# Sudo42b/vision.cpp

Hardware: AMD Instinct MI355X
Metric: images/sec, Depth-Anything-V2-Small 518x518 f16 (higher is better)
Workload: dtype f16; 1 GPU; Depth-Anything-V2-Small f16 (DINOv2-S ViT) 518x518 batch=32 per MI355X (BASELINE.json configs[1]); global_batch=32, weights=random-init synthetic GGUF (seed 0), parallelism=dp1 (image shards, no data-path collective), hip_graph=True

## Files before the change

### vision.cpp_amd/csrc/kernels_block16.hip

```cpp
#include "vx_common.h"

#include <cstdlib>
#include <type_traits>
#include <utility>

namespace {

constexpr int D = 384, HID = 1536;
constexpr int NT = D / 16;
constexpr int KB = D / 32;
constexpr int FR = 24;
constexpr int SLAB = FR * 1024;
constexpr int N_OUT = NT / 2;
constexpr int N_MLP = 2 * (HID / 32);
constexpr int N_QKV = 3 * NT / 2;

constexpr int V_BO = 0, V_G2 = 768, V_B2 = 1152, V_B1 = 1536, V_BFC2 = 3072;
constexpr int V_GN = 3840, V_BN = 4224, V_BQKV = 4608;
constexpr int V_GF = 5760, V_BF = 6144;
constexpr int V_TOTAL = 6528;

#ifndef VISP_BLOCK16_PF
#define VISP_BLOCK16_PF 4
#endif
#ifndef VISP_BLOCK16_DEFER
#define VISP_BLOCK16_DEFER 1
#endif
#ifndef VISP_BLOCK16_DEFER_MLP
#define VISP_BLOCK16_DEFER_MLP 0
#endif
#ifndef VISP_BLOCK16_LN_FENCE
#define VISP_BLOCK16_LN_FENCE 1
#endif
#ifndef VISP_BLOCK16_SPREAD
#define VISP_BLOCK16_SPREAD 1
#endif
constexpr int LN_FENCE = VISP_BLOCK16_LN_FENCE;
constexpr int SPREAD = VISP_BLOCK16_SPREAD;
constexpr int PF = VISP_BLOCK16_PF;
constexpr int DG = VISP_BLOCK16_DEFER;
static_assert(PF % 2 == 0 && FR % PF == 0 && PF - 2 * DG >= 2, "the window must hold the deferred groups and the next step's first group");
constexpr int SMEM_RING = 4 * SLAB;
constexpr int SMEM_BYTES = SMEM_RING + V_TOTAL * 4;
constexpr int WP = 2 * FR / 8;

typedef unsigned int u32x4 __attribute__((ext_vector_type(4)));
typedef unsigned int u32x2 __attribute__((ext_vector_type(2)));

template <int... I, class F>
__device__ __forceinline__ void static_for_impl(std::integer_sequence<int, I...>, F&& f) { (f(std::integral_constant<int, I>{}), ...); }
template <int N, class F>
__device__ __forceinline__ void static_for(F&& f) { static_for_impl(std::make_integer_sequence<int, N>{}, f); }
#define CI(x) (decltype(x)::value)

__device__ __forceinline__ float row_sum4(float v) {
    v += __shfl_xor(v, 16, 64);
    v += __shfl_xor(v, 32, 64);
    return v;
}

__device__ __forceinline__ void lds_dma16(const void* gsrc, unsigned lds_dst) {
    unsigned keep;
    asm volatile("s_mov_b32 %0, m0\n\ts_mov_b32 m0, %2\n\ts_nop 0\n\tglobal_load_lds_dwordx4 %1, off\n\ts_mov_b32 m0, %0"
                 : "=&s"(keep) : "v"(gsrc), "s"(lds_dst) : "memory");
}

#ifndef VISP_BLOCK16_DBG
#define VISP_BLOCK16_DBG 0
#endif
constexpr int DBG = VISP_BLOCK16_DBG;
#ifndef VISP_BLOCK16_MID
#define VISP_BLOCK16_MID 5
#endif

template <bool MLP, bool QKV, bool TAP>
__global__ __launch_bounds__(512) void dino_block16_kernel(const vx_dino_block_args args) {
    float* const a_x = args.x; const void* const a_att = args.att; const void* const a_wmlp = args.w_mlp; const void* const a_wqkv = args.w_qkv;
    const float* const a_vmlp = args.vec_mlp; const float* const a_vqkv = args.vec_qkv; const float* const a_vtap = args.vec_tap;
    void* const a_feat = args.feat; void* const a_q = args.q; void* const a_k = args.k; void* const a_v = args.v; float* const a_cap = args.cap_x1;
    const int a_M = args.M, a_T = args.T, a_H = args.H;
    const float a_qs = args.q_scale, a_eps = args.eps;
    unsigned long long* const a_stamps = static_cast<unsigned long long*>(args.stamps);
    auto stamp = [&](int slot) __attribute__((always_inline)) {
        if (a_stamps && threadIdx.x == 0) a_stamps[(size_t)blockIdx.x * 16 + slot] = slot >= 14 ? __builtin_amdgcn_s_memrealtime() : __builtin_amdgcn_s_memtime();
    };
    stamp(0);
    stamp(14);

    extern __shared__ __attribute__((aligned(16))) unsigned char smem[];
    unsigned char* const ring = smem;
    float* const vec = reinterpret_cast<float*>(smem + SMEM_RING);

    const int tid = threadIdx.x, lane = tid & 63;
    const int wave = __builtin_amdgcn_readfirstlane(tid >> 6);
    const int n = lane & 15, g = lane >> 4;
    const int m = blockIdx.x * 128 + wave * 16 + n;

    constexpr int row_bytes_f32 = D * 4, row_bytes_f16 = D * 2;
    const __amdgpu_buffer_rsrc_t rs_x = __builtin_amdgcn_make_buffer_rsrc(a_x, 0, (int)((long)a_M * row_bytes_f32), 0x00020000);
    const unsigned xoff = m < a_M ? (unsigned)m * row_bytes_f32 + 16 * g : 0x80000000u;
    auto ld_x = [&](int T) __attribute__((always_inline)) -> f32x4 {
        return __builtin_bit_cast(f32x4, __builtin_amdgcn_raw_buffer_load_b128(rs_x, xoff, 64 * T, 0));
    };
    auto st_x = [&](int T, f32x4 v) __attribute__((always_inline)) {
        __builtin_amdgcn_raw_buffer_store_b128(__builtin_bit_cast(u32x4, v), rs_x, xoff, 64 * T, 0);
    };

    auto pair_src = [&](int k) __attribute__((always_inline)) -> const unsigned char* {
        constexpr int first_qkv = MLP ? N_OUT + N_MLP : 0;
        const unsigned char* base = (MLP && k < first_qkv) ? static_cast<const unsigned char*>(a_wmlp) + (size_t)k * SLAB
                                                          : static_cast<const unsigned char*>(a_wqkv) + (size_t)(k - first_qkv) * SLAB;
        return base + (wave * WP) * 1024 + lane * 16;
    };
    constexpr int n_slabs = (MLP ? N_OUT + N_MLP : 0) + (QKV ? N_QKV : 0);
    const unsigned ring_lds = (unsigned)(size_t)(lptr_t)ring;
    auto feed_pair = [&](int k, int stage) __attribute__((always_inline)) {
        if constexpr (DBG & 1) return;
        const unsigned char* src = pair_src(k);
        const unsigned dst = __builtin_amdgcn_readfirstlane(ring_lds + stage * SLAB + wave * WP * 1024);
#pragma unroll
        for (int z = 0; z < WP; ++z) lds_dma16(src + z * 1024, dst + z * 1024);
    };
    const unsigned char* owed_src = nullptr;
    unsigned owed_dst = 0;
    bool owed = false;
    auto feed_piece = [&](int z) __attribute__((always_inline)) {
        if constexpr (DBG & 1) return;
        if (owed) lds_dma16(owed_src + z * 1024, owed_dst + z * 1024);
    };
    const unsigned char* const rd0 = ring + lane * 16;
    {
        feed_pair(0, 0);
        if constexpr (MLP)
            for (int i = tid; i < 3840 / 4; i += 512) reinterpret_cast<float4*>(vec)[i] = reinterpret_cast<const float4*>(a_vmlp)[i];
        if constexpr (QKV)
            for (int i = tid; i < 1920 / 4; i += 512) reinterpret_cast<float4*>(vec + V_GN)[i] = reinterpret_cast<const float4*>(a_vqkv)[i];
        if constexpr (TAP)
            for (int i = tid; i < 768 / 4; i += 512) reinterpret_cast<float4*>(vec + V_GF)[i] = reinterpret_cast<const float4*>(a_vtap)[i];
    }

    stamp(1);
    if constexpr ((DBG & 4096) != 0) { if (wave >= 4) __builtin_amdgcn_s_barrier(); }
    int k = 0, st = 0;
    const unsigned char *curx = rd0, *cury = rd0 + SLAB;
    f16x8 wfx[PF] = {}, wfy[PF] = {};

    unsigned long long w_vm = 0, w_bar = 0, w_n = 0;
    auto boundary = [&](auto yc, auto nfill) __attribute__((always_inline)) {
        constexpr int YOUNGER = CI(yc);
        if constexpr (DBG & 1024) {
            const unsigned long long t0 = __builtin_amdgcn_s_memtime();
            wait_vmcnt<YOUNGER>();
            const unsigned long long t1 = __builtin_amdgcn_s_memtime();
            __syncthreads();
            const unsigned long long t2 = __builtin_amdgcn_s_memtime();
            w_vm += t1 - t0; w_bar += t2 - t1; w_n += 1;
        } else {
        wait_vmcnt<YOUNGER>();
        if constexpr (!(DBG & 64)) __syncthreads();
        }
        curx = rd0 + st * SLAB;
        cury = curx + SLAB;
        if constexpr (!(DBG & 8)) {
#pragma unroll
            for (int i = 0; i < CI(nfill); ++i) {
                wfx[i] = *reinterpret_cast<const f16x8*>(curx + i * 1024);
                wfy[i] = *reinterpret_cast<const f16x8*>(cury + i * 1024);
            }
        }
        if constexpr (SPREAD) {
            owed = k + 2 < n_slabs;
            if (owed) {
                owed_src = pair_src(k + 2);
                owed_dst = __builtin_amdgcn_readfirstlane(ring_lds + (st ^ 2) * SLAB + wave * WP * 1024);
            }
        } else {
            if (k + 2 < n_slabs) feed_pair(k + 2, st ^ 2);
        }
        st ^= 2;
        k += 2;
    };
    auto stepx = [&](auto&& xm, auto&& ym, auto&& side, auto coldc, auto contc, auto yo, auto yc) __attribute__((always_inline)) {
        constexpr bool COLD = CI(coldc) != 0, CONT = CI(contc) != 0 && DG > 0;
        if constexpr (COLD || DG == 0) boundary(yo, std::integral_constant<int, PF>{});
        static_for<FR / 2>([&](auto gc) __attribute__((always_inline)) {
            constexpr int gi = CI(gc), f0 = 2 * gi, f1 = f0 + 1;
            if constexpr (CONT && gi == FR / 2 - DG) boundary(yc, std::integral_constant<int, PF - 2 * DG>{});
            if constexpr ((DBG & 2048) != 0 && gi == VISP_BLOCK16_MID) __builtin_amdgcn_s_barrier();
            ym(std::integral_constant<int, f1>{}, wfy[f1 % PF]);
            xm(std::integral_constant<int, f1>{}, wfx[f1 % PF]);
            ym(std::integral_constant<int, f0>{}, wfy[f0 % PF]);
            xm(std::integral_constant<int, f0>{}, wfx[f0 % PF]);
            constexpr int r0 = f0 + PF < FR ? f0 + PF : (CONT && gi >= FR / 2 - DG ? f0 + PF - FR : -1);
            if constexpr (r0 >= 0 && !(DBG & 8)) {
                wfx[f0 % PF] = *reinterpret_cast<const f16x8*>(curx + r0 * 1024);
                wfy[f0 % PF] = *reinterpret_cast<const f16x8*>(cury + r0 * 1024);
                wfx[f1 % PF] = *reinterpret_cast<const f16x8*>(curx + (r0 + 1) * 1024);
                wfy[f1 % PF] = *reinterpret_cast<const f16x8*>(cury + (r0 + 1) * 1024);
            }
            if constexpr (SPREAD && gi < WP) feed_piece(gi);
            side(std::integral_constant<int, 2 * f0>{});
            side(std::integral_constant<int, 2 * f0 + 1>{});
            side(std::integral_constant<int, 2 * f0 + 2>{});
            side(std::integral_constant<int, 2 * f0 + 3>{});
            __builtin_amdgcn_sched_barrier(0);
        });
    };
    constexpr std::integral_constant<int, 1> yes{};
    auto no_side = [](auto) {};
    constexpr std::integral_constant<int, 0> none{};

    auto vec4 = [&](const float* v, int T) __attribute__((always_inline)) -> f32x4 {
        const float4 q = *reinterpret_cast<const float4*>(v + 16 * T + 4 * g);
        f32x4 c = {q.x, q.y, q.z, q.w};
        return c;
    };
    auto mfma = [](const f16x8& w, const f16x8& b, f32x4 c) __attribute__((always_inline)) -> f32x4 {
        return __builtin_amdgcn_mfma_f32_16x16x32_f16(w, b, c, 0, 0, 0);
// ... 379 lines not shown
```

### vision.cpp_amd/csrc/kernels_gemm.hip

```cpp
#include "vx_common.h"

#include <algorithm>

extern "C" int vx_gemm_f16_raw(const vx_gemm_args* args, void* stream);

namespace {

constexpr int BK = 64;
constexpr int WAVE = 64;

__device__ __attribute__((aligned(16))) unsigned char g_zero_page[64];

constexpr bool epi_is_f16_tile(int epi) {
    return epi == VX_EPI_F16 || epi == VX_EPI_F16_GELU || epi == VX_EPI_F16_RELU || epi == VX_EPI_F16_ADD ||
           epi == VX_EPI_QKV || epi == VX_EPI_PIXSHUF || epi == VX_EPI_HEAD_OUT || epi == VX_EPI_LRELU_AGC ||
           epi == VX_EPI_SILU;
}

template <int BM, int BN, int WM, int WN, int STAGES, int EPI, bool CONV>
__global__ __launch_bounds__(64 * (BM / WM) * (BN / WN)) void gemm_kernel(const vx_gemm_args p) {
    constexpr int WAVES_N = BN / WN;
    constexpr int MI = WM / 32, NI = WN / 32;
    constexpr int NWAVES = (BM / WM) * WAVES_N;
    constexpr int THREADS = WAVE * NWAVES;
    constexpr int A_INSTR = BM / (8 * NWAVES);
    constexpr int B_INSTR = BN / (8 * NWAVES);
    static_assert(A_INSTR >= 1 && B_INSTR >= 1 && (128 * (BN / 8)) % THREADS == 0 && THREADS >= BM, "tile / wave layout");

    constexpr int STAGE_BYTES = (BM + BN) * BK * 2;
    constexpr int LOADS = A_INSTR + B_INSTR;
    extern __shared__ __attribute__((aligned(16))) unsigned char smem[];

    const int tid = threadIdx.x, lane = tid & 63;
    const int wave = __builtin_amdgcn_readfirstlane(tid >> 6);
    unsigned long long* const stamps = reinterpret_cast<unsigned long long*>(p.debug_stamps);
    auto stamp = [&](int slot) {
        if (stamps && tid == 0) stamps[(size_t)blockIdx.x * 8 + slot] = __builtin_amdgcn_s_memtime();
    };
    stamp(0);
    if (stamps && tid == 0) stamps[(size_t)blockIdx.x * 8 + 6] = __builtin_amdgcn_s_memrealtime();
    const int wr = wave / WAVES_N, wc = wave % WAVES_N;
    const int r = lane & 31, h = lane >> 5;

    const int n_tiles_n = p.N / BN;
    int tile;
    {
        const int nwg = gridDim.x, b = blockIdx.x;
        const int q = nwg >> 3, rem = nwg & 7, xcd = b & 7;
        tile = (xcd < rem ? xcd * (q + 1) : rem * (q + 1) + (xcd - rem) * q) + (b >> 3);
    }
    int ks = 0;
    if (p.k_splits > 1) {
        const int n_tiles = gridDim.x / p.k_splits;
        ks = tile / n_tiles;
        tile -= ks * n_tiles;
    }
    const int tile_m = tile / n_tiles_n, tile_n = tile - tile_m * n_tiles_n;
    const int m0 = tile_m * BM, n0 = tile_n * BN;
    int kbase = 0, nk = p.K / BK;
    if (p.k_splits > 1) {
        const int per = (nk + p.k_splits - 1) / p.k_splits;
        kbase = ks * per;
        nk = min(per, nk - kbase);
    }

    float* const s_bias = reinterpret_cast<float*>(smem + STAGES * STAGE_BYTES);
    float* const s_lambda = s_bias + BN;
    int* const s_pix = reinterpret_cast<int*>(s_lambda + BN);
    if constexpr (EPI == VX_EPI_F16_ADD) {
        if (p.win_ws > 0 && tid < BM) {
            const int m = m0 + tid;
            int pix = -1;
            if (m < p.M) {
                const int ws = p.win_ws, rw = p.win_res, rh = p.win_res_h > 0 ? p.win_res_h : p.win_res, N = ws * ws;
                const int nwx = (rw + ws - 1) / ws, nwy = (rh + ws - 1) / ws;
                const int in = m % N;
                int wq = m / N;
                const int wx = wq % nwx;
                wq /= nwx;
                const int wy = wq % nwy, bb = wq / nwy;
                int py = wy * ws + in / ws + p.win_shift, px = wx * ws + in % ws + p.win_shift;
                if (py >= nwy * ws) py -= nwy * ws;
                if (px >= nwx * ws) px -= nwx * ws;
                if (py < rh && px < rw) pix = (bb * rh + py) * rw + px;
            }
            s_pix[tid] = pix;
        }
    }
    if (tid < BN) {
        s_bias[tid] = p.bias ? p.bias[n0 + tid] : 0.0f;
        if constexpr (EPI == VX_EPI_RESID_F32 || EPI == VX_EPI_HEAD_OUT) s_lambda[tid] = p.lambda[n0 + tid];
    }

    const f16* __restrict__ Ag = reinterpret_cast<const f16*>(p.A);
    const f16* __restrict__ Wg = reinterpret_cast<const f16*>(p.W);

    const int l_row = lane >> 3, l_pos = lane & 7;
    long a_off[A_INSTR];
    const long a_pix = CONV ? (p.conv_pix > 0 ? p.conv_pix : p.conv_Cin) : 0;
    int a_iy0[A_INSTR], a_ix0[A_INSTR], a_chunk[A_INSTR];
#pragma unroll
    for (int i = 0; i < A_INSTR; ++i) {
        const int row = (wave * A_INSTR + i) * 8 + l_row;
        a_chunk[i] = swz128(row, l_pos);
        int m = m0 + row;
        if constexpr (CONV) {
            if (m < p.M) {
                int ohw = p.conv_OH * p.conv_OW;
                int b = m / ohw, rm = m - b * ohw;
                int oy = rm / p.conv_OW, ox = rm - oy * p.conv_OW;
                a_off[i] = (long)b * p.conv_H * p.conv_W * a_pix;
                a_iy0[i] = oy * p.conv_stride - p.conv_pad;
                a_ix0[i] = ox * p.conv_stride - p.conv_pad;
            } else {
                a_off[i] = -1;
                a_iy0[i] = a_ix0[i] = 0;
            }
        } else {
            if (m >= p.M) m = p.M - 1;
            long arow = m;
            if (p.a_group > 0) arow = (long)(m / p.a_group) * p.a_group_stride + p.a_row_off + (m % p.a_group);
            a_off[i] = arow * p.lda;
            a_iy0[i] = a_ix0[i] = 0;
        }
    }
    long b_off[B_INSTR];
    int b_chunk[B_INSTR];
#pragma unroll
    for (int i = 0; i < B_INSTR; ++i) {
        const int row = (wave * B_INSTR + i) * 8 + l_row;
        b_chunk[i] = swz128(row, l_pos);
        b_off[i] = (long)(n0 + row) * p.K;
    }
    const int cin8 = CONV ? (p.conv_Cin >> 3) : 1;
    const int ntaps = CONV ? p.conv_kh * p.conv_kw : 1;

    auto issue_loads = [&](int kt, int stage) {
        unsigned char* const sa = smem + stage * STAGE_BYTES;
        unsigned char* const sb = sa + BM * BK * 2;
        const int k0 = (kbase + kt) * BK;
#pragma unroll
        for (int i = 0; i < A_INSTR; ++i) {
            const f16* src;
            if constexpr (CONV) {
                src = reinterpret_cast<const f16*>(g_zero_page);
                int kc = (k0 >> 3) + a_chunk[i];
                int tap = kc / cin8, c8 = kc - tap * cin8;
                if (a_off[i] >= 0 && tap < ntaps) {
                    int ky = tap / p.conv_kw, kx = tap - ky * p.conv_kw;
                    int iy = a_iy0[i] + ky, ix = a_ix0[i] + kx;
                    if ((unsigned)iy < (unsigned)p.conv_H && (unsigned)ix < (unsigned)p.conv_W)
                        src = Ag + a_off[i] + ((long)iy * p.conv_W + ix) * a_pix + c8 * 8;
                }
            } else {
                src = Ag + a_off[i] + k0 + a_chunk[i] * 8;
            }
            __builtin_amdgcn_global_load_lds((gptr_t)src, (lptr_t)(sa + (wave * A_INSTR + i) * 1024), 16, 0, 0);
        }
#pragma unroll
        for (int i = 0; i < B_INSTR; ++i)
            __builtin_amdgcn_global_load_lds((gptr_t)(Wg + b_off[i] + k0 + b_chunk[i] * 8),
                                             (lptr_t)(sb + (wave * B_INSTR + i) * 1024), 16, 0, 0);
    };

    f32x16 acc[MI][NI];
#pragma unroll
    for (int mi = 0; mi < MI; ++mi)
#pragma unroll
        for (int ni = 0; ni < NI; ++ni)
#pragma unroll
            for (int e = 0; e < 16; ++e) acc[mi][ni][e] = 0.0f;

    int f_off[BK / 16];
#pragma unroll
    for (int ks = 0; ks < BK / 16; ++ks) f_off[ks] = r * 128 + swz128(r, ks * 2 + h) * 16;

    auto compute = [&](int stage) {
        const unsigned char* const sa = smem + stage * STAGE_BYTES + wr * WM * 128;
        const unsigned char* const sb = smem + stage * STAGE_BYTES + BM * BK * 2 + wc * WN * 128;
        f16x8 af[2][MI], bf[2][NI];
        auto load_frags = [&](int ks, int set) {
#pragma unroll
            for (int mi = 0; mi < MI; ++mi) af[set][mi] = *reinterpret_cast<const f16x8*>(sa + f_off[ks] + mi * 32 * 128);
#pragma unroll
            for (int ni = 0; ni < NI; ++ni) bf[set][ni] = *reinterpret_cast<const f16x8*>(sb + f_off[ks] + ni * 32 * 128);
        };
        load_frags(0, 0);
#pragma unroll
        for (int ks = 0; ks < BK / 16; ++ks) {
            const int set = ks & 1;
            if (ks + 1 < BK / 16) load_frags(ks + 1, set ^ 1);
            __builtin_amdgcn_sched_barrier(0);
            if constexpr (CONV) {
                if (p.a_relu) {
#pragma unroll
                    for (int mi = 0; mi < MI; ++mi)
#pragma unroll
                        for (int j = 0; j < 8; ++j) af[set][mi][j] = af[set][mi][j] > (f16)0 ? af[set][mi][j] : (f16)0;
                }
            }
#pragma unroll
            for (int mi = 0; mi < MI; ++mi)
#pragma unroll
                for (int ni = 0; ni < NI; ++ni)
                    acc[mi][ni] = __builtin_amdgcn_mfma_f32_32x32x16_f16(bf[set][ni], af[set][mi], acc[mi][ni], 0, 0, 0);
        }
    };
    auto barrier = [&]() {
        wait_lgkmcnt0();
        __builtin_amdgcn_s_barrier();
        asm volatile("" ::: "memory");
    };

    stamp(1);
    if constexpr (STAGES == 1) {
        issue_loads(0, 0);
        for (int kt = 0; kt < nk; ++kt) {
            wait_vmcnt<0>();
            barrier();
            if (kt == 0) stamp(2);
            compute(0);
            barrier();
            if (kt + 1 < nk) issue_loads(kt + 1, 0);
        }
    } else {
#pragma unroll
        for (int s = 0; s < STAGES - 1; ++s)
            if (s < nk) issue_loads(s, s);
        int stage = 0;
        for (int kt = 0; kt < nk; ++kt) {
            const int ahead = min(STAGES - 2, nk - 1 - kt);
            if (ahead >= 2) wait_vmcnt<2 * LOADS>();
            else if (ahead == 1) wait_vmcnt<LOADS>();
            else wait_vmcnt<0>();
            barrier();
            int next_stage = stage == 0 ? STAGES - 1 : stage - 1;
            if (kt + STAGES - 1 < nk) issue_loads(kt + STAGES - 1, next_stage);
            compute(stage);
            stage = stage + 1 == STAGES ? 0 : stage + 1;
        }
        barrier();
    }

    const int n_valid = p.n_valid > 0 ? p.n_valid : p.N;
    stamp(3);

    if (p.k_splits > 1) {
        float* const part = p.k_partial + (long)ks * p.M * p.N;
#pragma unroll
        for (int mi = 0; mi < MI; ++mi) {
            const int m = m0 + wr * WM + mi * 32 + r;
            if (m >= p.M) continue;
#pragma unroll
            for (int ni = 0; ni < NI; ++ni)
#pragma unroll
                for (int g = 0; g < 4; ++g) {
                    const float4 v = {acc[mi][ni][4 * g + 0], acc[mi][ni][4 * g + 1], acc[mi][ni][4 * g + 2], acc[mi][ni][4 * g + 3]};
                    *reinterpret_cast<float4*>(part + (long)m * p.N + n0 + wc * WN + ni * 32 + 8 * g + 4 * h) = v;
                }
        }
        return;
    }

    if constexpr (!epi_is_f16_tile(EPI)) {
#pragma unroll
        for (int mi = 0; mi < MI; ++mi) {
            const int m = m0 + wr * WM + mi * 32 + r;
            if (m >= p.M) continue;
            long row = m;
            int t = 0;
            if constexpr (EPI == VX_EPI_TOKENS) {
                int b = m / p.tokens_P;
                t = m - b * p.tokens_P;
                row = (long)b * (p.tokens_P + 1) + 1 + t;
            }
            float* xrow = reinterpret_cast<float*>(p.out) + row * p.ldo + n0;
            const float* add_row = nullptr;
            if constexpr (EPI == VX_EPI_RESID_F32) add_row = xrow;
            else add_row = p.pos + (long)(1 + t) * p.N + n0;
            float4 xin[NI][4];
#pragma unroll
            for (int ni = 0; ni < NI; ++ni)
#pragma unroll
                for (int g = 0; g < 4; ++g)
                    xin[ni][g] = *reinterpret_cast<const float4*>(add_row + wc * WN + ni * 32 + 8 * g + 4 * h);
#pragma unroll
            for (int ni = 0; ni < NI; ++ni) {
#pragma unroll
                for (int g = 0; g < 4; ++g) {
                    const int nl = wc * WN + ni * 32 + 8 * g + 4 * h;
                    const float4 bias = *reinterpret_cast<const float4*>(s_bias + nl);
                    float4 v = {acc[mi][ni][4 * g + 0] + bias.x, acc[mi][ni][4 * g + 1] + bias.y,
                                acc[mi][ni][4 * g + 2] + bias.z, acc[mi][ni][4 * g + 3] + bias.w};
                    float4 x = xin[ni][g];
                    if constexpr (EPI == VX_EPI_RESID_F32) {
                        const float4 lam = *reinterpret_cast<const float4*>(s_lambda + nl);
                        x.x += v.x * lam.x; x.y += v.y * lam.y; x.z += v.z * lam.z; x.w += v.w * lam.w;
                    } else {
                        x.x += v.x; x.y += v.y; x.z += v.z; x.w += v.w;
                    }
                    *reinterpret_cast<float4*>(xrow + nl) = x;
                }
            }
        }
    } else {
        constexpr int NCH16 = BN / 8;
        constexpr int PITCH = BN * 2;
        unsigned char* const st = smem;
        float out_scale = 1.0f;
        if constexpr (EPI == VX_EPI_QKV) out_scale = n0 < p.qkv_H * 64 ? p.q_scale : 1.0f;
        constexpr int MPP = (MI % 2 == 0 && BM / WM <= 2) ? 2 : 1;
        constexpr int PASSES = MI / MPP;
        constexpr int WPP = 32 * MPP;
        constexpr int STAGE_ROWS = (BM / WM) * WPP;
#pragma unroll
        for (int ps = 0; ps < PASSES; ++ps) {
        if (ps > 0) __syncthreads();
#pragma unroll
        for (int mp = 0; mp < MPP; ++mp) {
            const int mi = ps * MPP + mp;
            const int ml = wr * WPP + mp * 32 + r;
#pragma unroll
            for (int ni = 0; ni < NI; ++ni) {
#pragma unroll
                for (int g = 0; g < 4; ++g) {
                    const int nl = wc * WN + ni * 32 + 8 * g + 4 * h;
                    const float4 bias = *reinterpret_cast<const float4*>(s_bias + nl);
                    float v[4] = {acc[mi][ni][4 * g + 0] + bias.x, acc[mi][ni][4 * g + 1] + bias.y,
                                  acc[mi][ni][4 * g + 2] + bias.z, acc[mi][ni][4 * g + 3] + bias.w};
#pragma unroll
                    for (int j = 0; j < 4; ++j) {
                        if constexpr (EPI == VX_EPI_F16_GELU) v[j] = gelu_tanh(v[j]);
                        if constexpr (EPI == VX_EPI_F16_RELU || EPI == VX_EPI_HEAD_OUT) v[j] = fmaxf(v[j], 0.0f);
                        if constexpr (EPI == VX_EPI_F16_ADD) { if (p.relu) v[j] = fmaxf(v[j], 0.0f); }
                        if constexpr (EPI == VX_EPI_QKV) v[j] *= out_scale;
                        if constexpr (EPI == VX_EPI_SILU) v[j] = silu(v[j]);
                    }
                    if constexpr (EPI == VX_EPI_LRELU_AGC) {
                        const int m = m0 + wr * WM + ps * WPP + mp * 32 + r;
                        const float nz = (p.noise && m < p.M) ? p.noise[m % p.noise_hw] : 0.0f;
#pragma unroll
                        for (int j = 0; j < 4; ++j) {
                            const float t = v[j] + nz;
                            v[j] = fminf(fmaxf((t < 0.0f ? 0.2f * t : t) * 1.41421356f, -256.0f), 256.0f);
                        }
                    }
                    f16x4 o = {(f16)v[0], (f16)v[1], (f16)v[2], (f16)v[3]};
                    const int c8 = nl >> 2;
                    const int phys16 = (c8 >> 1) ^ (ml & (NCH16 - 1));
                    *reinterpret_cast<f16x4*>(st + ml * PITCH + phys16 * 16 + (c8 & 1) * 8) = o;
                }
            }
        }
        __syncthreads();
        if (ps == 0) stamp(4);
        constexpr int CHUNKS = STAGE_ROWS * NCH16;
        static_assert(CHUNKS % THREADS == 0, "staging read-out");
#pragma unroll
        for (int it = 0; it < CHUNKS / THREADS; ++it) {
            const int id = tid + it * THREADS;
            const int ml = id / NCH16, j = id % NCH16;
            const int m = m0 + (ml / WPP) * WM + ps * WPP + (ml % WPP), n = n0 + j * 8;
            if (m >= p.M || n >= n_valid) continue;
            f16x8 v = *reinterpret_cast<const f16x8*>(st + ml * PITCH + (j ^ (ml & (NCH16 - 1))) * 16);
            if constexpr (EPI == VX_EPI_HEAD_OUT) {
                float part = 0.0f;
#pragma unroll
                for (int q = 0; q < 8; ++q) part += (float)v[q] * s_lambda[j * 8 + q];
                part += __shfl_xor(part, 1, 64);
                part += __shfl_xor(part, 2, 64);
                if (j == 0) reinterpret_cast<float*>(p.out)[m] = fmaxf(part + p.head_bias, 0.0f) * p.head_scale;
            } else if constexpr (EPI == VX_EPI_F16 || EPI == VX_EPI_F16_GELU || EPI == VX_EPI_F16_RELU || EPI == VX_EPI_LRELU_AGC || EPI == VX_EPI_SILU) {
                if constexpr (EPI == VX_EPI_LRELU_AGC || EPI == VX_EPI_SILU) {
                    if (p.res1) {
                        const long ldr = (EPI == VX_EPI_SILU && p.ld_res1 > 0) ? p.ld_res1 : p.ldo;
                        const f16x8 a = *reinterpret_cast<const f16x8*>(reinterpret_cast<const f16*>(p.res1) + (long)m * ldr + n);
#pragma unroll
                        for (int q = 0; q < 8; ++q) v[q] = (f16)((float)v[q] + (float)a[q]);
                    }
                }
                *reinterpret_cast<f16x8*>(reinterpret_cast<f16*>(p.out) + (long)m * p.ldo + n) = v;
            } else if constexpr (EPI == VX_EPI_F16_ADD) {
                long o = (long)m * p.ldo + n;
                if (p.win_ws > 0) {
                    const int pix = s_pix[m - m0];
                    if (pix < 0) continue;
                    o = (long)pix * p.ldo + n;
                }
                if (p.res1) {
                    f16x8 a = *reinterpret_cast<const f16x8*>(reinterpret_cast<const f16*>(p.res1) + o);
                    if (p.res2) {
                        f16x8 b = *reinterpret_cast<const f16x8*>(reinterpret_cast<const f16*>(p.res2) + o);
#pragma unroll
                        for (int q = 0; q < 8; ++q) v[q] = (f16)((float)v[q] + (float)a[q] + (float)b[q]);
                    } else if (p.post_gelu) {
#pragma unroll
                        for (int q = 0; q < 8; ++q) v[q] = (f16)gelu_tanh((float)v[q] + (float)a[q]);
                    } else {
#pragma unroll
                        for (int q = 0; q < 8; ++q) v[q] = (f16)((float)v[q] + (float)a[q]);
                    }
                }
                *reinterpret_cast<f16x8*>(reinterpret_cast<f16*>(p.out) + o) = v;
            } else if constexpr (EPI == VX_EPI_QKV) {
                const int C = p.qkv_H * 64;
                const int which = n0 / C, cc = n - which * C;
                const int hh = cc >> 6, d = cc & 63;
                const int b0 = m0 / p.qkv_T;
                int b = b0 + (m >= (b0 + 1) * p.qkv_T ? 1 : 0);
                if (p.qkv_T < BM) b = m / p.qkv_T;
                const int t = m - b * p.qkv_T;
                f16* dst = reinterpret_cast<f16*>(which == 0 ? p.q : (which == 1 ? p.k : p.vt));
                *reinterpret_cast<f16x8*>(dst + (((long)b * p.qkv_H + hh) * p.qkv_T + t) * 64 + d) = v;
            } else if constexpr (EPI == VX_EPI_PIXSHUF) {
                const int s = p.ps_s;
                const int tap = n / p.ps_Cout, co = n - tap * p.ps_Cout;
                const int dy = tap / s, dx = tap - dy * s;
                const int hw = p.ps_H * p.ps_W;
                const int b = m / hw, rem = m - b * hw;
                const int y = rem / p.ps_W, x = rem - y * p.ps_W;
                const long o = (((long)b * p.ps_H * s + (y * s + dy)) * (p.ps_W * s) + (x * s + dx)) * p.ldo + co;
                *reinterpret_cast<f16x8*>(reinterpret_cast<f16*>(p.out) + o) = v;
            }
        }
        }
    }
    stamp(5);
    if (stamps && tid == 0) stamps[(size_t)blockIdx.x * 8 + 7] = __builtin_amdgcn_s_memrealtime();
}

template <int BM, int BN, int WM, int WN, int STAGES, int EPI, bool CONV>
int launch(const vx_gemm_args& a, hipStream_t s) {
    constexpr int ring = STAGES * (BM + BN) * BK * 2;
    constexpr int out_stage = epi_is_f16_tile(EPI) ? 128 * BN * 2 : 0;
    constexpr int smem = (ring > out_stage ? ring : out_stage) + 2 * BN * 4 + (EPI == VX_EPI_F16_ADD ? BM * 4 : 0);
    auto kern = gemm_kernel<BM, BN, WM, WN, STAGES, EPI, CONV>;
    if constexpr (smem > 48 * 1024) VX_CHECK(vx_ensure_dynamic_lds(reinterpret_cast<const void*>(kern), smem));
    int tiles_m = (a.M + BM - 1) / BM, tiles_n = a.N / BN;
    hipLaunchKernelGGL(kern, dim3(tiles_m * tiles_n * (a.k_splits > 1 ? a.k_splits : 1)), dim3(64 * (BM / WM) * (BN / WN)), smem, s, a);
    VX_LAUNCH_CHECK();
    return 1;
}

template <int EPI, bool CONV>
int dispatch_tile(const vx_gemm_args& a, hipStream_t s) {
    if (a.N % 128 == 0) {
        if constexpr (!CONV) {
            if (a.stages == 2) return launch<128, 128, 64, 64, 2, EPI, CONV>(a, s);
            if (a.stages == 4) return launch<256, 128, 128, 64, 1, EPI, CONV>(a, s);
            if (a.stages == 8) return launch<256, 128, 64, 64, 1, EPI, CONV>(a, s);
            if (a.stages == 16) return launch<128, 64, 64, 32, 1, EPI, CONV>(a, s);
            if (a.stages == 32) return launch<128, 128, 64, 32, 1, EPI, CONV>(a, s);
            if (a.stages == 64) return launch<192, 128, 96, 64, 1, EPI, CONV>(a, s);
            if (a.stages == 0) {
                const long n_t = a.N / 128;
                const long t128 = ((a.M + 127) / 128) * n_t, t192 = ((a.M + 191) / 192) * n_t;
                const long c128 = ((t128 + 1023) / 1024) * 128, c192 = ((t192 + 767) / 768) * 192;
                if (c192 < c128) return launch<192, 128, 96, 64, 1, EPI, CONV>(a, s);
            }
            return launch<128, 128, 64, 64, 1, EPI, CONV>(a, s);
        } else {
            return launch<128, 128, 64, 64, 1, EPI, CONV>(a, s);
        }
    }
    if (a.N % 64 == 0) return launch<128, 64, 64, 32, 1, EPI, CONV>(a, s);
    return launch<128, 32, 32, 32, 1, EPI, CONV>(a, s);
}

template <bool CONV>
int dispatch_epi(const vx_gemm_args& a, hipStream_t s) {
    switch (a.epi) {
        case VX_EPI_F16: return dispatch_tile<VX_EPI_F16, CONV>(a, s);
        case VX_EPI_F16_GELU: return dispatch_tile<VX_EPI_F16_GELU, CONV>(a, s);
        case VX_EPI_F16_RELU: return dispatch_tile<VX_EPI_F16_RELU, CONV>(a, s);
        case VX_EPI_F16_ADD: return dispatch_tile<VX_EPI_F16_ADD, CONV>(a, s);
        case VX_EPI_HEAD_OUT: return launch<128, 32, 32, 32, 1, VX_EPI_HEAD_OUT, CONV>(a, s);
        case VX_EPI_SILU: return dispatch_tile<VX_EPI_SILU, CONV>(a, s);
        default: break;
    }
    if constexpr (!CONV) {
        switch (a.epi) {
            case VX_EPI_RESID_F32: return dispatch_tile<VX_EPI_RESID_F32, false>(a, s);
            case VX_EPI_TOKENS: return dispatch_tile<VX_EPI_TOKENS, false>(a, s);
            case VX_EPI_QKV: return dispatch_tile<VX_EPI_QKV, false>(a, s);
            case VX_EPI_PIXSHUF: return dispatch_tile<VX_EPI_PIXSHUF, false>(a, s);
            case VX_EPI_LRELU_AGC: return dispatch_tile<VX_EPI_LRELU_AGC, false>(a, s);
            default: break;
        }
    }
    vx_set_error("vx_gemm_f16: unsupported epilogue %d (conv=%d)", a.epi, (int)CONV);
    return 0;
}

__global__ __launch_bounds__(256) void splitk_finish_kernel(const float* __restrict__ part, int S, long M, int N, const float* __restrict__ bias, int epi, int relu,
                                                            f16* __restrict__ out, long ldo, int n_valid, const f16* __restrict__ res1) {
    const int c8 = n_valid / 8;
    const long i = (long)blockIdx.x * 256 + threadIdx.x;
    if (i >= M * c8) return;
    const long m = i / c8;
    const int n = (int)(i - m * c8) * 8;
    float v[8];
#pragma unroll
    for (int j = 0; j < 8; ++j) v[j] = bias ? bias[n + j] : 0.0f;
    for (int s2 = 0; s2 < S; ++s2) {
        const float* p = part + ((long)s2 * M + m) * N + n;
        const float4 a = *reinterpret_cast<const float4*>(p), b = *reinterpret_cast<const float4*>(p + 4);
        v[0] += a.x; v[1] += a.y; v[2] += a.z; v[3] += a.w; v[4] += b.x; v[5] += b.y; v[6] += b.z; v[7] += b.w;
    }
    f16x8 o;
    if (epi == VX_EPI_F16_RELU || (epi == VX_EPI_F16_ADD && relu)) {
#pragma unroll
        for (int j = 0; j < 8; ++j) v[j] = fmaxf(v[j], 0.0f);
    }
    if (epi == VX_EPI_F16_ADD && res1) {
        const f16x8 rr = *reinterpret_cast<const f16x8*>(res1 + m * ldo + n);
#pragma unroll
        for (int j = 0; j < 8; ++j) v[j] += (float)rr[j];
    }
#pragma unroll
    for (int j = 0; j < 8; ++j) o[j] = (f16)v[j];
    *reinterpret_cast<f16x8*>(out + m * ldo + n) = o;
}

}

extern "C" int vx_gemm_pick_k_splits(int M, int N, int K) {
    const int bn = N % 128 == 0 ? 128 : (N % 64 == 0 ? 64 : 32);
    const long tiles = (long)((M + 127) / 128) * (N / bn);
    const int nk = K / BK;
    if (tiles >= 128 || nk < 16) return 1;
    int s = (int)std::min<long>(std::min(8, nk / 8), (256 + tiles - 1) / tiles);
    while (s > 1 && ((nk + s - 1) / s) * (s - 1) >= nk) --s;
    return s > 1 ? s : 1;
}

extern "C" int vx_gemm_f16(const vx_gemm_args* args, void* stream) {
    if (args->k_splits > 1) {
        vx_gemm_args a = *args;
        VX_REQUIRE(a.k_partial, "vx_gemm_f16: split-K needs the k_partial scratch (k_splits * M * N floats)");
        VX_REQUIRE(a.epi == VX_EPI_F16 || a.epi == VX_EPI_F16_RELU || (a.epi == VX_EPI_F16_ADD && !a.res2 && !a.post_gelu && a.win_ws == 0),
                   "vx_gemm_f16: split-K supports the F16, F16_RELU and plain F16_ADD epilogues");
        VX_REQUIRE(a.K % BK == 0 && a.k_splits <= a.K / BK && ((a.K / BK + a.k_splits - 1) / a.k_splits) * (a.k_splits - 1) < a.K / BK,
                   "vx_gemm_f16: k_splits = %d leaves an empty k range for K = %d", a.k_splits, a.K);
        const int nv = a.n_valid > 0 ? a.n_valid : a.N;
        VX_REQUIRE(nv % 8 == 0 && a.ldo % 8 == 0, "vx_gemm_f16: split-K output columns and row stride must be multiples of 8");
        const int epi = a.epi;
        const void* res1 = a.res1;
        a.epi = VX_EPI_F16;
        a.res1 = nullptr;
        a.k_splits = 0;
        vx_gemm_args g = a;
        g.k_splits = args->k_splits;
        if (!vx_gemm_f16_raw(&g, stream)) return 0;
        const long items = (long)a.M * (nv / 8);
        hipLaunchKernelGGL(splitk_finish_kernel, dim3((unsigned)((items + 255) / 256)), dim3(256), 0, as_stream(stream), a.k_partial, args->k_splits, (long)a.M, a.N, a.bias, epi, a.relu,
                           reinterpret_cast<f16*>(a.out), (long)a.ldo, nv, reinterpret_cast<const f16*>(res1));
        VX_LAUNCH_CHECK();
        return 1;
    }
    return vx_gemm_f16_raw(args, stream);
}

extern "C" int vx_gemm_f16_raw(const vx_gemm_args* args, void* stream) {
    const vx_gemm_args& a = *args;
    VX_REQUIRE(a.M > 0 && a.N > 0 && a.K > 0, "vx_gemm_f16: empty problem M=%d N=%d K=%d", a.M, a.N, a.K);
    VX_REQUIRE(a.K % BK == 0, "vx_gemm_f16: K=%d must be a multiple of %d (pad the weights)", a.K, BK);
    VX_REQUIRE(a.N % 32 == 0, "vx_gemm_f16: N=%d must be a multiple of 32", a.N);
    VX_REQUIRE(a.A && a.W, "vx_gemm_f16: null operand");
    const int nv = a.n_valid > 0 ? a.n_valid : a.N;
    if (a.epi == VX_EPI_RESID_F32 || a.epi == VX_EPI_TOKENS)
        VX_REQUIRE(nv >= a.N, "vx_gemm_f16: n_valid=%d < N=%d: the f32 epilogues store all N columns", nv, a.N);
    if (epi_is_f16_tile(a.epi)) {
        VX_REQUIRE(nv % 8 == 0, "vx_gemm_f16: n_valid=%d must be a multiple of 8 for f16 outputs", nv);
        VX_REQUIRE(a.epi == VX_EPI_QKV || a.epi == VX_EPI_HEAD_OUT || a.ldo % 8 == 0, "vx_gemm_f16: ldo=%ld must be a multiple of 8", (long)a.ldo);
    }
    if (a.epi == VX_EPI_PIXSHUF) VX_REQUIRE(a.ps_Cout % 8 == 0, "vx_gemm_f16: pixel-shuffle Cout=%d must be a multiple of 8", a.ps_Cout);
    if (a.epi == VX_EPI_QKV) VX_REQUIRE(a.N == 3 * a.qkv_H * 64, "vx_gemm_f16: QKV epilogue needs N == 3*H*64");
    if (a.post_gelu) VX_REQUIRE(a.epi == VX_EPI_F16_ADD && a.res1 && !a.res2, "vx_gemm_f16: post_gelu needs the F16_ADD epilogue with exactly one residual");
    if (a.win_ws > 0) {
        VX_REQUIRE(a.epi == VX_EPI_F16_ADD && a.conv_kh == 0 && a.win_res > 0, "vx_gemm_f16: window-order output needs the plain F16_ADD form");
        const long nw = (a.win_res + a.win_ws - 1) / a.win_ws, nwh = ((a.win_res_h > 0 ? a.win_res_h : a.win_res) + a.win_ws - 1) / a.win_ws;
        VX_REQUIRE(a.M % (nw * nwh * a.win_ws * a.win_ws) == 0, "vx_gemm_f16: M=%d is not a whole number of %ld x %ld window maps", a.M, nw, nwh);
        VX_REQUIRE(a.win_shift >= 0 && a.win_shift < a.win_ws && a.win_res_h >= 0, "vx_gemm_f16: bad window shift / height");
    }
    if (a.epi == VX_EPI_LRELU_AGC) VX_REQUIRE(!a.noise || a.noise_hw > 0, "vx_gemm_f16: lrelu_agc noise plane needs noise_hw > 0");
    if (a.epi == VX_EPI_HEAD_OUT) VX_REQUIRE(a.N == 32 && a.lambda, "vx_gemm_f16: head epilogue needs N == 32 and conv3 weights");
    if (a.ld_res1 != 0) VX_REQUIRE(a.epi == VX_EPI_SILU && a.ld_res1 % 8 == 0, "vx_gemm_f16: ld_res1=%ld needs the SiLU epilogue and a multiple of 8", (long)a.ld_res1);
    if (a.conv_kh > 0) {
        VX_REQUIRE(a.conv_Cin % 8 == 0, "vx_gemm_f16: conv Cin=%d must be a multiple of 8", a.conv_Cin);
        VX_REQUIRE(a.conv_pix == 0 || (a.conv_pix % 8 == 0 && a.conv_pix >= a.conv_Cin), "vx_gemm_f16: conv pixel stride %ld must be a multiple of 8 and >= Cin=%d",
                   (long)a.conv_pix, a.conv_Cin);
        VX_REQUIRE(a.K >= a.conv_kh * a.conv_kw * a.conv_Cin, "vx_gemm_f16: conv K too small");
        return dispatch_epi<true>(a, as_stream(stream));
    }
    VX_REQUIRE(a.conv_pix == 0, "vx_gemm_f16: conv_pix is an implicit-conv field");
    VX_REQUIRE(!a.a_relu, "vx_gemm_f16: a_relu is an implicit-conv field (the plain A loader has no ReLU)");
    VX_REQUIRE(a.lda % 8 == 0, "vx_gemm_f16: lda=%ld must be a multiple of 8", (long)a.lda);
    return dispatch_epi<false>(a, as_stream(stream));
}
```

### vision.cpp_amd/csrc/kernels_rcu.hip

```cpp
#include "vx_common.h"

#include <type_traits>

namespace {

constexpr int RC = 64;
constexpr int RPITCH = 144;
constexpr int RNW = 8;

struct rcu_geom {
    int TH, TW, ncx, ncy;
    int n_in, n_mid, n_out;
    int lds;
};

__host__ inline rcu_geom rcu_geometry(int H, int W) {
    rcu_geom g;
    g.ncx = (W + 19) / 20;
    g.TW = (W + g.ncx - 1) / g.ncx;
    int th = 320 / g.TW;
    if (th > H) th = H;
    g.ncy = (H + th - 1) / th;
    g.TH = (H + g.ncy - 1) / g.ncy;
    g.n_in = (g.TH + 4) * (g.TW + 4);
    g.n_mid = (g.TH + 2) * (g.TW + 2);
    g.n_out = g.TH * g.TW;
    g.lds = (g.n_in + ((g.n_mid + 31) & ~31)) * RPITCH + 4 * (RC * RC * 2) + 3 * RC * 4;
    return g;
}

constexpr int RSLAB = RC * RC * 2;
constexpr int RRING = 4;

template <bool PROJ>
__global__ __launch_bounds__(64 * RNW) void rcu_fused_kernel(const vx_rcu_args p, const int TH, const int TW, const int ncx, const int ncy) {
    extern __shared__ __attribute__((aligned(16))) unsigned char smem[];
    const int tid = threadIdx.x, lane = tid & 63;
    const int wave = __builtin_amdgcn_readfirstlane(tid >> 6);
    const int r = lane & 31, h = lane >> 5;
    const int H = p.H, W = p.W;
    const int IW = TW + 4, MW = TW + 2;
    const int n_in = (TH + 4) * IW, n_mid = (TH + 2) * MW, n_out = TH * TW;
    unsigned char* const s_in = smem;
    unsigned char* const s_mid = smem + n_in * RPITCH;
    unsigned char* const s_ring = s_mid + ((n_mid + 31) & ~31) * RPITCH;
    float* const s_bias = reinterpret_cast<float*>(s_ring + RRING * RSLAB);

    const int tile = blockIdx.x;
    const int b = tile / (ncx * ncy), trem = tile - b * (ncx * ncy);
    const int ty = trem / ncx, tx = trem - ty * ncx;
    const int y0 = ty * TH, x0 = tx * TW;

    constexpr int N_SLABS = PROJ ? 19 : 18;
    auto issue_slab = [&](int sl) {
        const unsigned char* src = sl < 9 ? reinterpret_cast<const unsigned char*>(p.w1) + sl * RSLAB
                                          : (sl < 18 ? reinterpret_cast<const unsigned char*>(p.w2) + (sl - 9) * RSLAB : reinterpret_cast<const unsigned char*>(p.wp));
        __builtin_amdgcn_global_load_lds((gptr_t)(src + wave * 1024 + lane * 16), (lptr_t)(s_ring + (sl & (RRING - 1)) * RSLAB + wave * 1024), 16, 0, 0);
    };

    if (tid < RC) {
        s_bias[tid] = p.b1 ? p.b1[tid] : 0.0f;
        s_bias[RC + tid] = p.b2 ? p.b2[tid] : 0.0f;
        s_bias[2 * RC + tid] = PROJ && p.bp ? p.bp[tid] : 0.0f;
    }

    issue_slab(0);
    issue_slab(1);
    issue_slab(2);

    {
        const f16* __restrict__ X = reinterpret_cast<const f16*>(p.x) + (long)b * H * W * RC;
        const int chunks = n_in * 8;
        constexpr int PER = 8;
        f16x8 v[PER];
#pragma unroll
        for (int i = 0; i < PER; ++i) {
            const int id = tid + i * 64 * RNW;
            const int pix = id >> 3, c = id & 7;
            const int ry = pix / IW, rx = pix - ry * IW;
            const int gy = y0 - 2 + ry, gx = x0 - 2 + rx;
            v[i] = f16x8{0, 0, 0, 0, 0, 0, 0, 0};
            if (id < chunks && (unsigned)gy < (unsigned)H && (unsigned)gx < (unsigned)W)
                v[i] = *reinterpret_cast<const f16x8*>(X + ((long)gy * W + gx) * RC + c * 8);
        }
        wait_vmcnt<0>();
#pragma unroll
        for (int i = 0; i < PER; ++i) {
            const int id = tid + i * 64 * RNW;
            if (id < chunks) *reinterpret_cast<f16x8*>(s_in + (id >> 3) * RPITCH + (id & 7) * 16) = v[i];
        }
    }
    const int w_off = r * 128 + ((h ^ ((r >> 1) & 7)) << 4);

    f32x16 acc[2][2];
    auto conv_stage = [&](auto first_slab, const unsigned char* src, int src_w, int dst_w, int n_dst, bool relu_in) {
        constexpr int S0 = decltype(first_slab)::value;
        const int n_mt = (n_dst + 31) >> 5;
        const bool any = wave < n_mt, two = wave + RNW < n_mt;
        int base[2];
#pragma unroll
        for (int mi = 0; mi < 2; ++mi) {
            int pd = (wave + mi * RNW) * 32 + r;
            if (pd >= n_dst) pd = 0;
            const int y = pd / dst_w, x = pd - y * dst_w;
            base[mi] = (y * src_w + x) * RPITCH + h * 16;
        }
#pragma unroll
        for (int mi = 0; mi < 2; ++mi)
#pragma unroll
            for (int ni = 0; ni < 2; ++ni)
#pragma unroll
                for (int e = 0; e < 16; ++e) acc[mi][ni][e] = 0.0f;
#pragma unroll
        for (int tap = 0; tap < 9; ++tap) {
            const int sl = S0 + tap;
            if (sl + 2 < N_SLABS) wait_vmcnt<2>();
            else if (sl + 1 < N_SLABS) wait_vmcnt<1>();
            else wait_vmcnt<0>();
            __syncthreads();
            if (sl + 3 < N_SLABS) issue_slab(sl + 3);
            if (!any) continue;
            const unsigned char* ws = s_ring + (sl & (RRING - 1)) * RSLAB;
            f16x8 wf[2][4];
#pragma unroll
            for (int ni = 0; ni < 2; ++ni)
#pragma unroll
                for (int ks = 0; ks < 4; ++ks) wf[ni][ks] = *reinterpret_cast<const f16x8*>(ws + ni * 4096 + (w_off ^ (ks << 5)));
            const int toff = ((tap / 3) * src_w + tap % 3) * RPITCH;
            auto one = [&](int mi) {
#pragma unroll
                for (int ks = 0; ks < 4; ++ks) {
                    f16x8 af = *reinterpret_cast<const f16x8*>(src + base[mi] + toff + ks * 32);
                    if (relu_in) {
#pragma unroll
                        for (int j = 0; j < 8; ++j) af[j] = af[j] > (f16)0 ? af[j] : (f16)0;
                    }
#pragma unroll
                    for (int ni = 0; ni < 2; ++ni) acc[mi][ni] = __builtin_amdgcn_mfma_f32_32x32x16_f16(wf[ni][ks], af, acc[mi][ni], 0, 0, 0);
                }
            };
            one(0);
            if (two) one(1);
        }
    };

    conv_stage(std::integral_constant<int, 0>{}, s_in, IW, MW, n_mid, true);
#pragma unroll
    for (int mi = 0; mi < 2; ++mi) {
        const int pd = (wave + mi * RNW) * 32 + r;
        if (pd >= n_mid) continue;
        const int y = pd / MW, x = pd - y * MW;
        const bool inside = (unsigned)(y0 - 1 + y) < (unsigned)H && (unsigned)(x0 - 1 + x) < (unsigned)W;
#pragma unroll
        for (int ni = 0; ni < 2; ++ni)
#pragma unroll
            for (int g = 0; g < 4; ++g) {
                const int nl = ni * 32 + 8 * g + 4 * h;
                const float4 bias = *reinterpret_cast<const float4*>(s_bias + nl);
                f16x4 o;
                o[0] = (f16)(inside ? fmaxf(acc[mi][ni][4 * g + 0] + bias.x, 0.0f) : 0.0f);
                o[1] = (f16)(inside ? fmaxf(acc[mi][ni][4 * g + 1] + bias.y, 0.0f) : 0.0f);
                o[2] = (f16)(inside ? fmaxf(acc[mi][ni][4 * g + 2] + bias.z, 0.0f) : 0.0f);
                o[3] = (f16)(inside ? fmaxf(acc[mi][ni][4 * g + 3] + bias.w, 0.0f) : 0.0f);
                *reinterpret_cast<f16x4*>(s_mid + pd * RPITCH + nl * 2) = o;
            }
    }

    conv_stage(std::integral_constant<int, 9>{}, s_mid, MW, TW, n_out, false);
    if constexpr (PROJ) __syncthreads();
    const f16* __restrict__ R2 = reinterpret_cast<const f16*>(p.res2);
    f16* __restrict__ O = reinterpret_cast<f16*>(p.out);
#pragma unroll
    for (int mi = 0; mi < 2; ++mi) {
        const int pd = (wave + mi * RNW) * 32 + r;
        if (pd >= n_out) continue;
        const int y = pd / TW, x = pd - y * TW;
        const int gy = y0 + y, gx = x0 + x;
        const bool inside = gy < H && gx < W;
        const long gpix = ((long)b * H + gy) * W + gx;
        const unsigned char* xin = s_in + ((y + 2) * IW + x + 2) * RPITCH;
#pragma unroll
        for (int ni = 0; ni < 2; ++ni)
#pragma unroll
            for (int g = 0; g < 4; ++g) {
                const int nl = ni * 32 + 8 * g + 4 * h;
                const float4 bias = *reinterpret_cast<const float4*>(s_bias + RC + nl);
                const f16x4 xs = *reinterpret_cast<const f16x4*>(xin + nl * 2);
                float v[4] = {acc[mi][ni][4 * g + 0] + bias.x, acc[mi][ni][4 * g + 1] + bias.y, acc[mi][ni][4 * g + 2] + bias.z, acc[mi][ni][4 * g + 3] + bias.w};
                f16x4 o = {(f16)v[0], (f16)v[1], (f16)v[2], (f16)v[3]};
                o = o + xs;
                if (R2 && inside) o = o + *reinterpret_cast<const f16x4*>(R2 + gpix * RC + nl);
                if constexpr (PROJ) *reinterpret_cast<f16x4*>(s_mid + pd * RPITCH + nl * 2) = o;
                else if (inside) *reinterpret_cast<f16x4*>(O + gpix * RC + nl) = o;
            }
    }
    if constexpr (!PROJ) return;

    {
        wait_vmcnt<0>();
        __syncthreads();
        const int n_mt = (n_out + 31) >> 5;
        if (wave >= n_mt) return;
        const bool two = wave + RNW < n_mt;
        f16x8 wf[2][4];
#pragma unroll
        for (int ni = 0; ni < 2; ++ni)
#pragma unroll
            for (int ks = 0; ks < 4; ++ks) wf[ni][ks] = *reinterpret_cast<const f16x8*>(s_ring + (18 & (RRING - 1)) * RSLAB + ni * 4096 + (w_off ^ (ks << 5)));
#pragma unroll
        for (int mi = 0; mi < 2; ++mi) {
            if (mi == 1 && !two) break;
            int pd = (wave + mi * RNW) * 32 + r;
            const bool have = pd < n_out;
            if (!have) pd = 0;
            f32x16 a2[2];
#pragma unroll
            for (int ni = 0; ni < 2; ++ni)
#pragma unroll
                for (int e = 0; e < 16; ++e) a2[ni][e] = 0.0f;
#pragma unroll
            for (int ks = 0; ks < 4; ++ks) {
                const f16x8 af = *reinterpret_cast<const f16x8*>(s_mid + pd * RPITCH + ks * 32 + h * 16);
#pragma unroll
                for (int ni = 0; ni < 2; ++ni) a2[ni] = __builtin_amdgcn_mfma_f32_32x32x16_f16(wf[ni][ks], af, a2[ni], 0, 0, 0);
            }
            const int y = pd / TW, x = pd - y * TW;
            const int gy = y0 + y, gx = x0 + x;
            if (!have || gy >= H || gx >= W) continue;
            const long gpix = ((long)b * H + gy) * W + gx;
#pragma unroll
            for (int ni = 0; ni < 2; ++ni)
#pragma unroll
                for (int g = 0; g < 4; ++g) {
                    const int nl = ni * 32 + 8 * g + 4 * h;
                    const float4 bias = *reinterpret_cast<const float4*>(s_bias + 2 * RC + nl);
                    f16x4 o = {(f16)(a2[ni][4 * g + 0] + bias.x), (f16)(a2[ni][4 * g + 1] + bias.y), (f16)(a2[ni][4 * g + 2] + bias.z), (f16)(a2[ni][4 * g + 3] + bias.w)};
                    *reinterpret_cast<f16x4*>(O + gpix * RC + nl) = o;
                }
        }
    }
}

}

extern "C" int vx_rcu_supported(int H, int W) {
    if (H < 1 || W < 1 || H > 96 || W > 96) return 0;
    const rcu_geom g = rcu_geometry(H, W);
    return g.n_in <= 512 && g.n_mid <= 512 && g.n_out <= 512 && g.lds <= 160 * 1024;
}

extern "C" int vx_rcu_fused_f16(const vx_rcu_args* args, void* stream) {
    const vx_rcu_args& a = *args;
    VX_REQUIRE(a.B > 0, "vx_rcu_fused_f16: empty batch");
    VX_REQUIRE(vx_rcu_supported(a.H, a.W),
               "vx_rcu_fused_f16: map %d x %d is not built (1..96 per side, and a tile whose three regions hold at most 512 pixels and fit 160 KB of LDS)", a.W, a.H);
    VX_REQUIRE(a.x && a.w1 && a.w2 && a.out, "vx_rcu_fused_f16: missing operands");
    const rcu_geom g = rcu_geometry(a.H, a.W);
    const long blocks = (long)a.B * g.ncx * g.ncy;
    VX_REQUIRE(blocks < (1l << 30), "vx_rcu_fused_f16: too many tiles");
    if (a.wp) {
        VX_CHECK(vx_ensure_dynamic_lds(reinterpret_cast<const void*>(&rcu_fused_kernel<true>), g.lds));
        hipLaunchKernelGGL((rcu_fused_kernel<true>), dim3((unsigned)blocks), dim3(64 * RNW), g.lds, as_stream(stream), a, g.TH, g.TW, g.ncx, g.ncy);
    } else {
        VX_CHECK(vx_ensure_dynamic_lds(reinterpret_cast<const void*>(&rcu_fused_kernel<false>), g.lds));
        hipLaunchKernelGGL((rcu_fused_kernel<false>), dim3((unsigned)blocks), dim3(64 * RNW), g.lds, as_stream(stream), a, g.TH, g.TW, g.ncx, g.ncy);
    }
    VX_LAUNCH_CHECK();
    return 1;
}
```

### vision.cpp_amd/csrc/vx_device.h

```cpp
#pragma once

typedef __attribute__((address_space(1))) const void* gptr_t;
typedef __attribute__((address_space(3))) void* lptr_t;

__device__ __forceinline__ float wave_sum(float v) {
#pragma unroll
    for (int o = 32; o > 0; o >>= 1) v += __shfl_xor(v, o, 64);
    return v;
}
__device__ __forceinline__ float wave_max(float v) {
#pragma unroll
    for (int o = 32; o > 0; o >>= 1) v = fmaxf(v, __shfl_xor(v, o, 64));
    return v;
}
__device__ __forceinline__ float wave_min(float v) {
#pragma unroll
    for (int o = 32; o > 0; o >>= 1) v = fminf(v, __shfl_xor(v, o, 64));
    return v;
}

__device__ __forceinline__ float gelu_tanh(float x) {
    const float c1 = -2.0f * 0.79788456080286535588f * 1.44269504088896340736f;
    const float c3 = c1 * 0.044715f;
    const float w = fmaf(x * x, c3, c1);
    return x * __builtin_amdgcn_rcpf(1.0f + __builtin_amdgcn_exp2f(x * w));
}

__device__ __forceinline__ float silu(float x) {
    return x * __builtin_amdgcn_rcpf(1.0f + __builtin_amdgcn_exp2f(x * -1.44269504088896340736f));
}

__device__ __forceinline__ float relu1(float x) { return __int_as_float(max(__float_as_int(x), 0)); }

__device__ __forceinline__ float other_half(float v) {
    const unsigned u = __float_as_uint(v);
    auto r = __builtin_amdgcn_permlane32_swap(u, u, false, false);
    return __uint_as_float((threadIdx.x & 32) ? r[0] : r[1]);
}

__device__ __forceinline__ int swz128(int row, int chunk) { return chunk ^ ((row >> 1) & 7); }

template <int N>
__device__ __forceinline__ void wait_vmcnt() { asm volatile("s_waitcnt vmcnt(%0)" ::"n"(N) : "memory"); }
__device__ __forceinline__ void wait_lgkmcnt0() { asm volatile("s_waitcnt lgkmcnt(0)" ::: "memory"); }

__device__ __forceinline__ f16x8 residue_pixel(const float (&v)[3]) {
    f16x8 o = {0, 0, 0, 0, 0, 0, 0, 0};
#pragma unroll
    for (int c = 0; c < 3; ++c) {
        const f16 hi = (f16)v[c];
        o[c] = hi;
        o[3 + c] = (f16)(v[c] - (float)hi);
    }
    return o;
}
```

Before: 6521 images/s.

## Use inline-asm LDS DMA and lightweight barriers; enable 2-stage GEMM ring selectively

Result: no change. 6574 images/s, median of 5 (+0.8%).

```diff
diff --git a/vision.cpp_amd/csrc/kernels_block16.hip b/vision.cpp_amd/csrc/kernels_block16.hip
--- a/vision.cpp_amd/csrc/kernels_block16.hip
+++ b/vision.cpp_amd/csrc/kernels_block16.hip
@@ -59,11 +59,6 @@
     return v;
 }
 
-__device__ __forceinline__ void lds_dma16(const void* gsrc, unsigned lds_dst) {
-    unsigned keep;
-    asm volatile("s_mov_b32 %0, m0\n\ts_mov_b32 m0, %2\n\ts_nop 0\n\tglobal_load_lds_dwordx4 %1, off\n\ts_mov_b32 m0, %0"
-                 : "=&s"(keep) : "v"(gsrc), "s"(lds_dst) : "memory");
-}
 
 #ifndef VISP_BLOCK16_DBG
 #define VISP_BLOCK16_DBG 0
diff --git a/vision.cpp_amd/csrc/kernels_gemm.hip b/vision.cpp_amd/csrc/kernels_gemm.hip
--- a/vision.cpp_amd/csrc/kernels_gemm.hip
+++ b/vision.cpp_amd/csrc/kernels_gemm.hip
@@ -135,9 +135,12 @@
     const int cin8 = CONV ? (p.conv_Cin >> 3) : 1;
     const int ntaps = CONV ? p.conv_kh * p.conv_kw : 1;
 
+    const unsigned smem_lds = lds_addr(smem);
+    auto copy16 = [&](const f16* src, int stage, int piece) {
+        if constexpr (STAGES > 1) lds_dma16(src, __builtin_amdgcn_readfirstlane(smem_lds + stage * STAGE_BYTES + piece * 1024));
+        else __builtin_amdgcn_global_load_lds((gptr_t)src, (lptr_t)(smem + stage * STAGE_BYTES + piece * 1024), 16, 0, 0);
+    };
     auto issue_loads = [&](int kt, int stage) {
-        unsigned char* const sa = smem + stage * STAGE_BYTES;
-        unsigned char* const sb = sa + BM * BK * 2;
         const int k0 = (kbase + kt) * BK;
 #pragma unroll
         for (int i = 0; i < A_INSTR; ++i) {
@@ -155,12 +158,10 @@
             } else {
                 src = Ag + a_off[i] + k0 + a_chunk[i] * 8;
             }
-            __builtin_amdgcn_global_load_lds((gptr_t)src, (lptr_t)(sa + (wave * A_INSTR + i) * 1024), 16, 0, 0);
-        }
-#pragma unroll
-        for (int i = 0; i < B_INSTR; ++i)
-            __builtin_amdgcn_global_load_lds((gptr_t)(Wg + b_off[i] + k0 + b_chunk[i] * 8),
-                                             (lptr_t)(sb + (wave * B_INSTR + i) * 1024), 16, 0, 0);
+            copy16(src, stage, wave * A_INSTR + i);
+        }
+#pragma unroll
+        for (int i = 0; i < B_INSTR; ++i) copy16(Wg + b_off[i] + k0 + b_chunk[i] * 8, stage, BM * BK * 2 / 1024 + wave * B_INSTR + i);
     };
 
     f32x16 acc[MI][NI];
@@ -442,6 +443,11 @@
     return 1;
 }
 
+int gemm_ring_env() {
+    static const int ring = getenv("VISP_GEMM_RING") ? atoi(getenv("VISP_GEMM_RING")) : 0;
+    return ring;
+}
+
 template <int EPI, bool CONV>
 int dispatch_tile(const vx_gemm_args& a, hipStream_t s) {
     if (a.N % 128 == 0) {
@@ -458,8 +464,13 @@
                 const long c128 = ((t128 + 1023) / 1024) * 128, c192 = ((t192 + 767) / 768) * 192;
                 if (c192 < c128) return launch<192, 128, 96, 64, 1, EPI, CONV>(a, s);
             }
+            if (gemm_ring_env() == 2) return launch<128, 128, 64, 64, 2, EPI, CONV>(a, s);
+            if constexpr (EPI == VX_EPI_TOKENS) {
+                if (gemm_ring_env() != 1) return launch<128, 128, 64, 64, 2, EPI, CONV>(a, s);
+            }
             return launch<128, 128, 64, 64, 1, EPI, CONV>(a, s);
         } else {
+            if (gemm_ring_env() == 2 || (gemm_ring_env() != 1 && a.conv_stride > 1 && a.K >= 3456)) return launch<128, 128, 64, 64, 2, EPI, CONV>(a, s);
             return launch<128, 128, 64, 64, 1, EPI, CONV>(a, s);
         }
     }
diff --git a/vision.cpp_amd/csrc/kernels_rcu.hip b/vision.cpp_amd/csrc/kernels_rcu.hip
--- a/vision.cpp_amd/csrc/kernels_rcu.hip
+++ b/vision.cpp_amd/csrc/kernels_rcu.hip
@@ -52,10 +52,11 @@
     const int y0 = ty * TH, x0 = tx * TW;
 
     constexpr int N_SLABS = PROJ ? 19 : 18;
+    const unsigned ring_lds = lds_addr(s_ring);
     auto issue_slab = [&](int sl) {
         const unsigned char* src = sl < 9 ? reinterpret_cast<const unsigned char*>(p.w1) + sl * RSLAB
                                           : (sl < 18 ? reinterpret_cast<const unsigned char*>(p.w2) + (sl - 9) * RSLAB : reinterpret_cast<const unsigned char*>(p.wp));
-        __builtin_amdgcn_global_load_lds((gptr_t)(src + wave * 1024 + lane * 16), (lptr_t)(s_ring + (sl & (RRING - 1)) * RSLAB + wave * 1024), 16, 0, 0);
+        lds_dma16(src + wave * 1024 + lane * 16, __builtin_amdgcn_readfirstlane(ring_lds + (sl & (RRING - 1)) * RSLAB + wave * 1024));
     };
 
     if (tid < RC) {
@@ -117,7 +118,7 @@
             if (sl + 2 < N_SLABS) wait_vmcnt<2>();
             else if (sl + 1 < N_SLABS) wait_vmcnt<1>();
             else wait_vmcnt<0>();
-            __syncthreads();
+            ring_barrier();
             if (sl + 3 < N_SLABS) issue_slab(sl + 3);
             if (!any) continue;
             const unsigned char* ws = s_ring + (sl & (RRING - 1)) * RSLAB;
@@ -167,7 +168,7 @@
     }
 
     conv_stage(std::integral_constant<int, 9>{}, s_mid, MW, TW, n_out, false);
-    if constexpr (PROJ) __syncthreads();
+    if constexpr (PROJ) ring_barrier();
     const f16* __restrict__ R2 = reinterpret_cast<const f16*>(p.res2);
     f16* __restrict__ O = reinterpret_cast<f16*>(p.out);
 #pragma unroll
@@ -198,7 +199,7 @@
 
     {
         wait_vmcnt<0>();
-        __syncthreads();
+        ring_barrier();
         const int n_mt = (n_out + 31) >> 5;
         if (wave >= n_mt) return;
         const bool two = wave + RNW < n_mt;
diff --git a/vision.cpp_amd/csrc/vx_device.h b/vision.cpp_amd/csrc/vx_device.h
--- a/vision.cpp_amd/csrc/vx_device.h
+++ b/vision.cpp_amd/csrc/vx_device.h
@@ -44,6 +44,19 @@
 __device__ __forceinline__ void wait_vmcnt() { asm volatile("s_waitcnt vmcnt(%0)" ::"n"(N) : "memory"); }
 __device__ __forceinline__ void wait_lgkmcnt0() { asm volatile("s_waitcnt lgkmcnt(0)" ::: "memory"); }
 
+
+__device__ __forceinline__ void lds_dma16(const void* gsrc, unsigned lds_dst) {
+    unsigned keep;
+    asm volatile("s_mov_b32 %0, m0\n\ts_mov_b32 m0, %2\n\ts_nop 0\n\tglobal_load_lds_dwordx4 %1, off\n\ts_mov_b32 m0, %0"
+                 : "=&s"(keep) : "v"(gsrc), "s"(lds_dst) : "memory");
+}
+__device__ __forceinline__ unsigned lds_addr(const void* p) { return (unsigned)(size_t)(lptr_t)p; }
+__device__ __forceinline__ void ring_barrier() {
+    asm volatile("s_waitcnt lgkmcnt(0)" ::: "memory");
+    __builtin_amdgcn_s_barrier();
+    asm volatile("" ::: "memory");
+}
+
 __device__ __forceinline__ f16x8 residue_pixel(const float (&v)[3]) {
     f16x8 o = {0, 0, 0, 0, 0, 0, 0, 0};
 #pragma unroll
```
